# yangdongchao/Text-to-sound-Synthesis

Hardware: AMD Instinct MI355X
Metric: 10s clips/sec whole-node, 100-step Diffsound sample + VQ decode + vocoder (higher is better)
Workload: dtype f32 via 2-way fp16 split (3 MFMA passes, fp32 accumulate); 1 GPU; BASELINE configs[2]: full pipeline, batch 64 per GPU, 100 diffusion steps, codebook 256: CLIP text tower -> 19-layer denoiser -> SpecVQGAN decode -> MelGAN 22 kHz; global_batch=64, n_layer=19, parallelism=caption-sharded x1

## Files before the change

### include/diffsound_hip.h

```cpp
#ifndef DIFFSOUND_HIP_H
#define DIFFSOUND_HIP_H
#include <stdint.h>
#ifdef __cplusplus
extern "C" {
#endif

typedef void* ds_stream_t;

int ds_version(void);
const char* ds_last_error_string(void);

enum { DS_LOAD_DENSE = 0, DS_LOAD_CONV2D = 1, DS_LOAD_CONV1D = 2, DS_LOAD_CONVT1D = 3 };
enum { DS_PRO_NONE = 0, DS_PRO_AFFINE = 1, DS_PRO_AFFINE_SWISH = 2, DS_PRO_LRELU = 3 };
enum { DS_ACT_NONE = 0, DS_ACT_GELU2 = 1, DS_ACT_TANH = 2 };
enum { DS_STORE_ROW = 0, DS_STORE_BATCH_T = 1, DS_STORE_CONVT = 2, DS_STORE_ATTN = 3 };

typedef struct ds_gemm_desc {
    const float* A;
    const float* W;
    const float* bias;
    const float* R;
    float* C;
    int32_t M, N, K;
    int32_t lda, ldw, ldc, ldr;
// ... 15 lines not shown
    int64_t a_plane, c_plane;
    void* attn_kv;
    int32_t attn_heads, attn_nkey;
    int64_t attn_qplane;
} ds_gemm_desc;

int ds_gemm(const ds_gemm_desc* d, ds_stream_t stream);
void ds_gemm_force_tile(int cfg);
int ds_gemm_f16x2(const ds_gemm_desc* d, ds_stream_t stream);
int ds_gemm_f16x2_multi(const ds_gemm_desc* descs, int n, int cfg, ds_stream_t stream);
int ds_conv2d_f16x2(const ds_gemm_desc* d, ds_stream_t stream);
void ds_gemm_f16x2_force_tile(int cfg);
int ds_gemm_f16x2_auto_tile(int M, int N, int groups);
void ds_gemm_f16x2_set_balance_slots(int slots);
int ds_gemm_f16x2_plan(int cfg, int M, int N, int store, int* m_off, int* nbig, int* nsmall);

int ds_embed(const int64_t* tokens, const float* emb, const float* pos, float* out, int M, int L, int D,
             ds_stream_t stream);
int ds_adaln(const float* x, float* y, int M, int L, int D, const float* table, const int64_t* t,
             ds_stream_t stream);
int ds_layernorm(const float* x, float* y, int M, int D, const float* gamma, const float* beta,
                 ds_stream_t stream);
int ds_attention(const float* q, int ldq, const float* k, int ldk, const float* v, int ldv, float* o, int ldo,
                 int B, int heads, int Lq, int Lk, float scale, ds_stream_t stream);

int ds_attention_ex(const float* q, int ldq, const float* k, int ldk, const float* v, int ldv, float* o, int ldo,
                    int B, int heads, int Lq, int Lk, float scale, int causal, int f16_round, ds_stream_t stream);
int ds_attention_f16x2(const float* q, int ldq, const float* k, int ldk, const float* v, int ldv, float* o, int ldo,
                       int B, int heads, int Lq, int Lk, float scale, ds_stream_t stream);
int ds_adaln_split(const float* x, void* yh, int M, int L, int D, const float* table, const int64_t* t,
                   ds_stream_t stream);
int ds_layernorm_split(const float* x, void* yh, int M, int D, const float* gamma, const float* beta,
                       ds_stream_t stream);
int ds_attention_f16x2_split(const float* q, int ldq, const float* k, int ldk, const float* v, int ldv, void* oh,
                             int ldo, int B, int heads, int Lq, int Lk, float scale, ds_stream_t stream);
int ds_attn_nkey(int Lk);
int ds_attention_f16x2_ready(const void* qh, long long q_plane, const void* kv_img, void* oh, int ldo, int B, int heads,
                             int Lq, int Lk, float scale, ds_stream_t stream);
int ds_attn_pack_kv(const float* kv, int ld, int v_col, void* img, int B, int heads, int Lk, ds_stream_t stream);
int ds_embed_f16(const int64_t* tokens, const float* emb, const float* pos, float* out, int M, int L, int D,
                 ds_stream_t stream);
int ds_layernorm_f16(const float* x, float* y, int M, int D, const float* gamma, const float* beta,
                     ds_stream_t stream);
int ds_l2norm_rows_f16(const float* x, float* y, int M, int D, ds_stream_t stream);

int ds_sample_tail(const float* logits, const int64_t* xt, const int64_t* t, const float* u, const float* sched,
                   int64_t* out_tokens, float* dbg_log_pred, float* dbg_trunc, float* dbg_post, int B, int L,
                   int K, int T, int initial, float trunc_r, ds_stream_t stream);

int ds_sample_tail_ex(const float* logits, const int64_t* xt, const int64_t* t, const float* u, const float* sched,
                      int64_t* out_tokens, float* dbg_log_pred, float* dbg_trunc, float* dbg_post, int B, int L,
                      int K, int T, int initial, float trunc_r, int trunc_k, ds_stream_t stream);

int ds_q_sample(const int64_t* x0, const int64_t* t, const float* u, const float* sched, int64_t* out_tokens, int B,
                int L, int K, int T, ds_stream_t stream);

int ds_philox_uniforms(const int64_t* gids, unsigned long long seed, int call, int rng_stream, float* u, int B, int L,
                       int K, ds_stream_t stream);
int ds_sample_tail_rng(const float* logits, const int64_t* xt, const int64_t* t, const int64_t* gids,
                       unsigned long long seed, int call, const float* sched, int64_t* out_tokens, int B, int L, int K,
                       int T, int initial, float trunc_r, int trunc_k, ds_stream_t stream);
int ds_q_sample_rng(const int64_t* x0, const int64_t* t, const int64_t* gids, unsigned long long seed, int call,
                    const float* sched, int64_t* out_tokens, int B, int L, int K, int T, ds_stream_t stream);

int ds_sample_tail_hold(const float* logits, const int64_t* xt, const int64_t* t, const float* u, const float* sched,
                        int64_t* out_tokens, float* dbg_log_pred, float* dbg_trunc, float* dbg_post, int B, int L, int K,
// ... 283 lines not shown
```

### text-to-sound-synthesis_amd/_lib.py

```python
import ctypes as C
import os

import torch

_HERE = os.path.dirname(os.path.abspath(__file__))
LIB_PATH = os.environ.get("DIFFSOUND_LIB") or os.path.join(_HERE, "libdiffsound_hip.so")

LOAD_DENSE, LOAD_CONV2D, LOAD_CONV1D, LOAD_CONVT1D = 0, 1, 2, 3
PRO_NONE, PRO_AFFINE, PRO_AFFINE_SWISH, PRO_LRELU = 0, 1, 2, 3
ACT_NONE, ACT_GELU2, ACT_TANH = 0, 1, 2
LEVEL_MEASURE, LEVEL_PEAK, LEVEL_RMS, LEVEL_LOUDNESS = 0, 1, 2, 3
PASTE_EQUAL_POWER, PASTE_LINEAR = 0, 1
STORE_ROW, STORE_BATCH_T, STORE_CONVT, STORE_ATTN = 0, 1, 2, 3
(LP_ADALN1, LP_W_QKV, LP_B_QKV, LP_W_PROJ1, LP_B_PROJ1, LP_ADALN2, LP_W_Q2, LP_B_Q2, LP_W_KV2, LP_B_KV2,
 LP_W_PROJ2, LP_B_PROJ2, LP_LN2_G, LP_LN2_B, LP_W_FC1, LP_B_FC1, LP_W_FC2, LP_B_FC2, LP_COUNT) = range(19)

_vp, _i32, _i64, _f = C.c_void_p, C.c_int32, C.c_int64, C.c_float


class GemmDesc(C.Structure):
    _fields_ = [("A", _vp), ("W", _vp), ("bias", _vp), ("R", _vp), ("C", _vp),
                ("M", _i32), ("N", _i32), ("K", _i32),
                ("lda", _i32), ("ldw", _i32), ("ldc", _i32), ("ldr", _i32),
                ("groups", _i32),
# ... 9 lines not shown

class DenoiserDesc(C.Structure):
    _fields_ = [("n_layer", _i32), ("n_embd", _i32), ("n_head", _i32), ("seq_len", _i32),
                ("cond_len", _i32), ("cond_dim", _i32), ("n_codes", _i32), ("n_steps", _i32),
                ("mlp_mult", _i32),
                ("tok_emb", _vp), ("pos_emb", _vp), ("lnf_g", _vp), ("lnf_b", _vp),
                ("w_logits", _vp), ("b_logits", _vp), ("sched", _vp)]


_PROTOS = {
    "ds_version": (C.c_int, []),
    "ds_last_error_string": (C.c_char_p, []),
    "ds_gemm": (C.c_int, [C.POINTER(GemmDesc), _vp]),
    "ds_gemm_force_tile": (None, [C.c_int]),
    "ds_gemm_f16x2": (C.c_int, [C.POINTER(GemmDesc), _vp]),
    "ds_conv2d_f16x2": (C.c_int, [C.POINTER(GemmDesc), _vp]),
    "ds_gemm_f16x2_multi": (C.c_int, [C.POINTER(GemmDesc), C.c_int, C.c_int, _vp]),
    "ds_gemm_f16x2_auto_tile": (C.c_int, [C.c_int, C.c_int, C.c_int]),
    "ds_gemm_f16x2_force_tile": (None, [C.c_int]),
    "ds_gemm_f16x2_set_balance_slots": (None, [C.c_int]),
    "ds_gemm_f16x2_plan": (C.c_int, [C.c_int, C.c_int, C.c_int, C.c_int, C.POINTER(C.c_int), C.POINTER(C.c_int), C.POINTER(C.c_int)]),
    "ds_denoiser_set_split_weights": (C.c_int, [_vp, C.c_int, C.POINTER(_vp), C.POINTER(_f), _vp, _f]),
    "ds_embed": (C.c_int, [_vp, _vp, _vp, _vp, C.c_int, C.c_int, C.c_int, _vp]),
    "ds_adaln": (C.c_int, [_vp, _vp, C.c_int, C.c_int, C.c_int, _vp, _vp, _vp]),
    "ds_layernorm": (C.c_int, [_vp, _vp, C.c_int, C.c_int, _vp, _vp, _vp]),
    "ds_attention": (C.c_int, [_vp, C.c_int, _vp, C.c_int, _vp, C.c_int, _vp, C.c_int,
                               C.c_int, C.c_int, C.c_int, C.c_int, _f, _vp]),
    "ds_attention_ex": (C.c_int, [_vp, C.c_int, _vp, C.c_int, _vp, C.c_int, _vp, C.c_int,
                                  C.c_int, C.c_int, C.c_int, C.c_int, _f, C.c_int, C.c_int, _vp]),
    "ds_attention_f16x2": (C.c_int, [_vp, C.c_int, _vp, C.c_int, _vp, C.c_int, _vp, C.c_int,
                                     C.c_int, C.c_int, C.c_int, C.c_int, _f, _vp]),
    "ds_adaln_split": (C.c_int, [_vp, _vp, C.c_int, C.c_int, C.c_int, _vp, _vp, _vp]),
    "ds_layernorm_split": (C.c_int, [_vp, _vp, C.c_int, C.c_int, _vp, _vp, _vp]),
    "ds_attention_f16x2_split": (C.c_int, [_vp, C.c_int, _vp, C.c_int, _vp, C.c_int, _vp, C.c_int,
                                           C.c_int, C.c_int, C.c_int, C.c_int, _f, _vp]),
    "ds_attn_nkey": (C.c_int, [C.c_int]),
    "ds_attention_f16x2_ready": (C.c_int, [_vp, _i64, _vp, _vp, C.c_int, C.c_int, C.c_int, C.c_int, C.c_int, _f, _vp]),
    "ds_attn_pack_kv": (C.c_int, [_vp, C.c_int, C.c_int, _vp, C.c_int, C.c_int, C.c_int, _vp]),
    "ds_embed_f16": (C.c_int, [_vp, _vp, _vp, _vp, C.c_int, C.c_int, C.c_int, _vp]),
    "ds_layernorm_f16": (C.c_int, [_vp, _vp, C.c_int, C.c_int, _vp, _vp, _vp]),
    "ds_l2norm_rows_f16": (C.c_int, [_vp, _vp, C.c_int, C.c_int, _vp]),
    "ds_sample_tail": (C.c_int, [_vp, _vp, _vp, _vp, _vp, _vp, _vp, _vp, _vp,
                                 C.c_int, C.c_int, C.c_int, C.c_int, C.c_int, _f, _vp]),
    "ds_sample_tail_ex": (C.c_int, [_vp, _vp, _vp, _vp, _vp, _vp, _vp, _vp, _vp,
                                    C.c_int, C.c_int, C.c_int, C.c_int, C.c_int, _f, C.c_int, _vp]),
    "ds_q_sample": (C.c_int, [_vp, _vp, _vp, _vp, _vp, C.c_int, C.c_int, C.c_int, C.c_int, _vp]),
    "ds_philox_uniforms": (C.c_int, [_vp, C.c_uint64, C.c_int, C.c_int, _vp, C.c_int, C.c_int, C.c_int, _vp]),
    "ds_sample_tail_rng": (C.c_int, [_vp, _vp, _vp, _vp, C.c_uint64, C.c_int, _vp, _vp, C.c_int, C.c_int, C.c_int, C.c_int,
                                     C.c_int, _f, C.c_int, _vp]),
    "ds_q_sample_rng": (C.c_int, [_vp, _vp, _vp, C.c_uint64, C.c_int, _vp, _vp, C.c_int, C.c_int, C.c_int, C.c_int, _vp]),
    "ds_vq_argmin": (C.c_int, [_vp, _vp, _vp, _vp, _vp, C.c_int, C.c_int, C.c_int, _vp]),
    "ds_loss_tail": (C.c_int, [_vp, _vp, _vp, _vp, _vp, _vp, _vp, _vp, _vp, C.c_int, C.c_int, C.c_int, C.c_int, _vp]),
    "ds_loss_tail_bwd": (C.c_int, [_vp, _vp, _vp, _vp, _vp, _vp, _vp, C.c_int, C.c_int, C.c_int, C.c_int, _f, _f, _f,
                                   C.c_int, _vp]),
    "ds_layernorm_bwd": (C.c_int, [_vp, _vp, _vp, _vp, C.c_int, C.c_int, C.c_int, C.c_int, _vp, _vp, _vp, _vp]),
    "ds_layernorm_bwd_chunks": (C.c_int, [C.c_int, C.c_int, C.c_int]),
    "ds_layernorm_bwd_sums": (C.c_int, [_vp, _vp, _vp, _vp, C.c_int, C.c_int, C.c_int, C.c_int, _vp, _vp, _vp, C.c_int, _vp]),
    "ds_colsum": (C.c_int, [_vp, _vp, C.c_int, C.c_int, C.c_int, _i64, _i64, C.c_int, _vp]),
    "ds_colsum_ws": (C.c_int, [_vp, _vp, C.c_int, C.c_int, C.c_int, _i64, _i64, C.c_int, _vp, _i64, _vp]),
    "ds_gelu2": (C.c_int, [_vp, _vp, _vp, _i64, _vp]),
    "ds_softmax_bwd_rows": (C.c_int, [_vp, _vp, C.c_int, C.c_int, C.c_int, _f, _vp]),
    "ds_attention_bwd": (C.c_int, [_vp, C.c_int, _vp, C.c_int, _vp, C.c_int, _vp, C.c_int, _vp, C.c_int, _vp, C.c_int,
                                   _vp, C.c_int, _vp, C.c_int, _vp, C.c_int, C.c_int, C.c_int, C.c_int, _f, _vp]),
    "ds_attention_bwd_f16x2": (C.c_int, [_vp, C.c_int, _vp, C.c_int, _vp, C.c_int, _vp, C.c_int, _vp, C.c_int, _vp, C.c_int,
                                   _vp, C.c_int, _vp, C.c_int, _vp, C.c_int, C.c_int, C.c_int, C.c_int, _f, _vp]),
    "ds_attention_bwd_f16x2_mon": (C.c_int, [_vp, C.c_int, _vp, C.c_int, _vp, C.c_int, _vp, C.c_int, _vp, C.c_int, _vp, C.c_int,
# ... 275 lines not shown
```

### text-to-sound-synthesis_amd/csrc/api.hip

```cpp
#include <stdarg.h>
#include <stdio.h>
#include <string.h>

#include <vector>

#include "sampler.h"

static thread_local char g_err[512] = "";

void ds_set_error(const char* fmt, ...) {
    va_list ap;
    va_start(ap, fmt);
    vsnprintf(g_err, sizeof(g_err), fmt, ap);
    va_end(ap);
}

extern "C" int ds_version(void) { return 100; }
extern "C" const char* ds_last_error_string(void) { return g_err; }

static void fill(GemmParams& p, const ds_gemm_desc* d) {
    p.A = d->A; p.W = d->W; p.bias = d->bias; p.R = d->R; p.C = d->C;
    p.M = d->M; p.N = d->N; p.K = d->K;
    p.lda = d->lda; p.ldw = d->ldw > 0 ? d->ldw : d->K; p.ldc = d->ldc; p.ldr = d->ldr;
    p.groups = d->groups > 0 ? d->groups : 1;
// ... 93 lines not shown
    DS_CHECK_ARG(w_logits3, "missing split logits weight");
    h->lp3.assign(split3, split3 + (size_t)h->d.n_layer * DS_LP_COUNT);
    h->osc.assign(out_scales, out_scales + (size_t)h->d.n_layer * DS_LP_COUNT);
    h->w_logits3 = w_logits3;
    h->logits_osc = logits_scale;
    h->split_mode = mode;
    return 0;
}

extern "C" int ds_denoiser_create(const ds_denoiser_desc* desc, const void* const* layer_ptrs, ds_denoiser** out) {
    DS_CHECK_ARG(desc && layer_ptrs && out, "null pointer");
    DS_CHECK_ARG(desc->n_embd == 1024 && desc->n_embd == desc->n_head * 64, "built for n_embd 1024, head dim 64");
    DS_CHECK_ARG(desc->n_codes == 256 || desc->n_codes == 512, "codebook size must be 256 or 512");
    DS_CHECK_ARG(desc->cond_dim % 32 == 0 && desc->cond_len <= 96 && desc->seq_len <= 288, "unsupported lengths");
    DS_CHECK_ARG(desc->tok_emb && desc->pos_emb && desc->lnf_g && desc->lnf_b && desc->w_logits && desc->b_logits &&
                     desc->sched,
                 "null weight pointer");
    for (int i = 0; i < desc->n_layer * DS_LP_COUNT; ++i) DS_CHECK_ARG(layer_ptrs[i], "null layer pointer");
    ds_denoiser* h = new ds_denoiser;
    h->d = *desc;
    h->lp.resize((size_t)desc->n_layer * DS_LP_COUNT);
    for (size_t i = 0; i < h->lp.size(); ++i) h->lp[i] = (const float*)layer_ptrs[i];
    *out = h;
    return 0;
}

extern "C" void ds_denoiser_destroy(ds_denoiser* h) { delete h; }

struct Carve {
    float *x, *hn, *qkv, *att, *fc, *logits;
    float* kvimg;
};
static size_t attn_img_floats(int B, int heads, int Lk) { return (size_t)B * heads * 4 * ds_attn_nkey(Lk) * 64 / 2; }
static const int PS_ROWS = 272;
bool ds_gemm_f16x2_ps_taken(int B, int N);
static int rows_per_sample(const ds_denoiser* h, int B) {
    const int L = h->d.seq_len;
    if (!h->pad_rows || h->split_mode != DS_SPLIT_F16X2 || L > PS_ROWS || L <= PS_ROWS - 16) return L;
    return ds_gemm_f16x2_ps_taken(B, h->d.n_embd) ? PS_ROWS : L;
}
extern "C" int ds_denoiser_rows_per_sample(const ds_denoiser* h, int B) { return h && B > 0 ? rows_per_sample(h, B) : -1; }
extern "C" int ds_denoiser_set_row_padding(ds_denoiser* h, int on) {
    DS_CHECK_ARG(h, "null handle");
    h->pad_rows = on != 0;
    return 0;
}

int ds_amax_packed_hi(const void* plane, int M, int K, float* out, ds_stream_t stream);
extern "C" int ds_denoiser_set_range_monitor(ds_denoiser* h, float* peak) {
    DS_CHECK_ARG(h, "null handle");
    h->range_peak = peak;
    return 0;
}

static size_t carve(const ds_denoiser* h, int B, void* ws, Carve* c, int Lp = 0) {
    const size_t M = (size_t)B * (Lp > 0 ? Lp : PS_ROWS > h->d.seq_len ? PS_ROWS : h->d.seq_len), D = h->d.n_embd;
    const size_t M16 = (M + 15) & ~(size_t)15;
    size_t off = 0;
    auto take = [&](size_t n) {
        float* p = ws ? (float*)ws + off : nullptr;
        off += (n + 63) & ~(size_t)63;
        return p;
    };
    Carve t;
    t.x = take(M * D);
    t.hn = take(M16 * D);
// ... 91 lines not shown
        int rc_ = (x);    \
        if (rc_) return rc_; \
    } while (0)

extern "C" int ds_denoiser_cond_kv(const ds_denoiser* h, const float* cond, int B, float* kv, ds_stream_t stream) {
    DS_CHECK_ARG(h && cond && kv && B > 0, "bad arguments");
    const int D = h->d.n_embd, Mc = B * h->d.cond_len;
    if (h->split_mode == DS_SPLIT_F16X2) {
        const size_t per = kv_layer_img_floats(h, B);
        float* rows = kv + (size_t)h->d.n_layer * per;
        for (int l = 0; l < h->d.n_layer; ++l) {
            TRY(dense(cond, h->d.cond_dim, h->P(l, DS_LP_W_KV2), h->P(l, DS_LP_B_KV2), nullptr, rows, 2 * D, Mc, 2 * D,
                      h->d.cond_dim, DS_ACT_NONE, (hipStream_t)stream));
            TRY(ds_attn_pack_kv(rows, 2 * D, D, kv + (size_t)l * per, B, h->d.n_head, h->d.cond_len, stream));
        }
        return 0;
    }
    for (int l = 0; l < h->d.n_layer; ++l)
        TRY(dense(cond, h->d.cond_dim, h->P(l, DS_LP_W_KV2), h->P(l, DS_LP_B_KV2), nullptr,
                  kv + (size_t)l * Mc * 2 * D, 2 * D, Mc, 2 * D, h->d.cond_dim, DS_ACT_NONE, (hipStream_t)stream));
    return 0;
}

static int forward_impl(const ds_denoiser* h, const int64_t* tokens, const int64_t* t, const float* kv, int B,
                        const Carve& w, float* logits, int layout, hipStream_t s, int Lp, bool zero_kv_pad = true) {
    const ds_denoiser_desc& d = h->d;
    const int D = d.n_embd, Lv = d.seq_len, L = Lp, M = B * L, Mc = B * d.cond_len, F = D * d.mlp_mult;
    DS_CHECK_ARG(Lp == Lv || (layout == 0 && Lp > Lv), "padded rows need the row-major logits layout");
    g_prof_row_frac = (double)Lv / Lp;
    const float scale = 0.125f;
    const bool f16 = h->split_mode == DS_SPLIT_F16X2;
    const long long M16 = (M + 15) & ~15;
    const long long pD = f16 ? M16 * D : 0, pF = f16 ? M16 * F : 0;
    auto adaln = [&](int l, int slot) {
        return f16 ? ds_adaln_split(w.x, w.hn, M, L, D, h->P(l, slot), t, s)
                   : ds_adaln(w.x, w.hn, M, L, D, h->P(l, slot), t, s);
    };
    auto lnorm = [&](const float* g, const float* b_) {
        return f16 ? ds_layernorm_split(w.x, w.hn, M, D, g, b_, s) : ds_layernorm(w.x, w.hn, M, D, g, b_, s);
    };
    auto attn = [&](const float* q, int ldq, const float* k, const float* v, int ldkv, int Lk) {
        return ds_attention(q, ldq, k, ldkv, v, ldkv, w.att, D, B, d.n_head, L, Lk, scale, s);
    };
    const long long qpl = (long long)M * D;
    const int nkS = ds_attn_nkey(L);
    auto lin_attn = [&](int l, int slot, int bslot, int N, int n_weight, void* imgs) {
        return dense(w.hn, D, h->P(l, slot), h->P(l, bslot), nullptr, w.qkv, N, M, N, D, DS_ACT_NONE, s, DS_STORE_ATTN, L,
                     h->P3(l, slot), h->split_mode, h->S3(l, slot), pD, 0, imgs, d.n_head, nkS, qpl,
                     (long long)n_weight * D);
    };
    auto attn_ready = [&](const void* imgs, int Lk) {
        return ds_attention_f16x2_ready(w.qkv, qpl, imgs, w.att, D, B, d.n_head, L, Lk, scale, s);
    };
    if (f16 && zero_kv_pad) {
        hipError_t e = hipMemsetAsync(w.kvimg, 0, attn_img_floats(B, d.n_head, L) * sizeof(float), s);
        if (e != hipSuccess) {
            ds_set_error("forward: hipMemsetAsync: %s", hipGetErrorString(e));
            return -2;
        }
    }
    auto lin = [&](int l, int slot, int bslot, const float* A, int lda, long long ap, const float* R, float* C, int N,
                   int K, int act, long long cp) {
        return dense(A, lda, h->P(l, slot), h->P(l, bslot), R, C, N, M, N, K, act, s, DS_STORE_ROW, L, h->P3(l, slot),
                     h->split_mode, h->S3(l, slot), ap, cp);
    };
    TRY(ds_embed_rows(tokens, d.tok_emb, d.pos_emb, w.x, B, Lv, L, D, s));
    for (int l = 0; l < d.n_layer; ++l) {
        TRY(adaln(l, DS_LP_ADALN1));
        if (f16) {
            TRY(lin_attn(l, DS_LP_W_QKV, DS_LP_B_QKV, 3 * D, 3 * D, w.kvimg));
            TRY(attn_ready(w.kvimg, Lv));
        } else {
// ... 371 lines not shown
```

### text-to-sound-synthesis_amd/csrc/gemm_f16x2_ps.hip

```cpp
#include <stdlib.h>

#include "common.h"


typedef _Float16 h8 __attribute__((ext_vector_type(8)));
typedef unsigned u32x4 __attribute__((ext_vector_type(4)));
typedef unsigned u32x2 __attribute__((ext_vector_type(2)));
typedef __attribute__((address_space(1))) const void* ds_gptr;
typedef __attribute__((address_space(3))) void* ds_lptr;

#define PS_HLD 32
#define PS_BM 288
#define PS_BN 256
#define PS_LEAD 6
#define PS_GM 4
#define PS_STAGE_BYTES (2 * 2 * (PS_BM + PS_BN) * PS_HLD * 2)
#define PS_EPI_BYTES (2 * 64 * (PS_BN + 4) * 4)
#ifndef PS_DIRECT_SPLIT
#define PS_DIRECT_SPLIT 1
#endif
#ifndef PS_DIRECT_QK
#define PS_DIRECT_QK 0
#endif
#define PS_LDS_BYTES (PS_EPI_BYTES > PS_STAGE_BYTES ? PS_EPI_BYTES : PS_STAGE_BYTES)
#define PS_SIG(q_) ((0x78 >> (2 * (q_))) & 3)

enum { PS_EPI_ROW = 0, PS_EPI_SPLIT = 1, PS_EPI_ATTN = 2 };

template <int EPI, bool NB16>
__global__ __launch_bounds__(512, 1) void ds_gemm_f16x2_ps_kernel(const GemmParams p) {
    extern __shared__ __attribute__((aligned(16))) unsigned char smem_raw[];
    constexpr int BM = PS_BM, BN = PS_BN, HLD = PS_HLD, LEAD = PS_LEAD;
    constexpr int APL = BM * HLD, BPL = BN * HLD, STAGE = 2 * (APL + BPL);
    _Float16* smem = (_Float16*)smem_raw;
    const int tid = threadIdx.x, lane = tid & 63, wave = tid >> 6, l31 = lane & 31, hh = lane >> 5;
    const int wr = wave >> 2, wc = wave & 3;
    const int L = p.rows_per_sample;
    const int tiles_n = p.N / BN, nblk = gridDim.x;
    int bid = blockIdx.x;
    {
        const int xcd = bid & 7, idx = bid >> 3, q = nblk >> 3, r = nblk & 7;
        bid = (xcd < r ? xcd * (q + 1) : r * (q + 1) + (xcd - r) * q) + idx;
    }
    int tm_, tn_;
    {
        const int tiles_m = p.M / L;
        const int per = PS_GM * tiles_n, grp = bid / per, first = grp * PS_GM;
        const int gsz = tiles_m - first < PS_GM ? tiles_m - first : PS_GM;
        const int in = bid - grp * per;
        tm_ = first + in % gsz;
        tn_ = in / gsz;
    }
    const int row_lo = tm_ * L;
    const int m0 = (row_lo >> 4) << 4, n0 = tn_ * BN;
    const int nk = p.K / 32;
    const _Float16* Ap = (const _Float16*)p.A;
    const _Float16* Wp = (const _Float16*)p.W;
    unsigned long long src[4][2], src8;
    int ldsoff[4][2], ldsoff8;
    const unsigned lane16 = lane * 16;
    const int rgsA = (p.M + 15) >> 4, rgsB = (p.N + 15) >> 4;
#define PS_BASE(dst_, ptr_)                                                                          \
    do {                                                                                             \
        const unsigned long long a_ = (unsigned long long)(ptr_);                                    \
        dst_ = ((unsigned long long)(unsigned)__builtin_amdgcn_readfirstlane((unsigned)(a_ >> 32)) << 32) | \
               (unsigned long long)(unsigned)__builtin_amdgcn_readfirstlane((unsigned)a_);           \
    } while (0)
#pragma unroll
    for (int ty = 0; ty < 4; ++ty)
#pragma unroll
        for (int k = 0; k < 2; ++k) {
            const int idx = 2 * wave + k, plane = idx >> 3, r = idx & 7;
            const bool isA = (ty == 0 || ty == 3);
            const int s = isA ? (ty == 3) : (ty == 2);
            const int gip = isA ? (r >> 2) * 8 + s * 4 + (r & 3)
                                : (r >> 1) * 4 + s * 2 + (r & 1);
            int rg = ((isA ? m0 : n0) >> 4) + gip;
            const int rgs = isA ? rgsA : rgsB;
            if (rg >= rgs) rg = rgs - 1;
            PS_BASE(src[ty][k], (isA ? Ap + plane * p.a_plane : Wp + plane * p.w3_plane) + (size_t)rg * nk * 512);
            ldsoff[ty][k] = __builtin_amdgcn_readfirstlane((isA ? plane * 18 + gip : 36 + plane * 16 + gip) * 1024);
        }
    {
        const int e = wave & 3, plane = e >> 1, gip = 16 + (e & 1);
        int rg = (m0 >> 4) + gip;
        if (rg >= rgsA) rg = rgsA - 1;
        PS_BASE(src8, Ap + plane * p.a_plane + (size_t)rg * nk * 512);
        ldsoff8 = __builtin_amdgcn_readfirstlane((plane * 18 + gip) * 1024);
    }
#define PS_ISSUE(tile_, ty_, buf_)                                                                   \
    do {                                                                                             \
        _Pragma("unroll") for (int k = 0; k < 2; ++k)                                                \
            __builtin_amdgcn_global_load_lds((ds_gptr)((const unsigned char*)(src[ty_][k] + (unsigned long long)(tile_) * 1024) + lane16), \
                                             (ds_lptr)(smem_raw + (buf_) * (STAGE * 2) + ldsoff[ty_][k]), 16, 0, 0); \
        if ((ty_) == 3)                                                                              \
            __builtin_amdgcn_global_load_lds((ds_gptr)((const unsigned char*)(src8 + (unsigned long long)(tile_) * 1024) + lane16), \
                                             (ds_lptr)(smem_raw + (buf_) * (STAGE * 2) + ldsoff8), 16, 0, 0); \
    } while (0)
#define PS_DMA_ASM(base_, lds_, stage_)                                                              \
    do {                                                                                             \
        asm volatile("s_add_u32 m0, %2, %3\n\ts_nop 0\n\tglobal_load_lds_dwordx4 %0, %1"            \
                     :: "v"(lane16), "s"(base_), "s"(lds_), "n"(stage_) : "memory", "scc", "m0");    \
        base_ += 1024;                                                                               \
    } while (0)
#define PS_ISSUE_LOOP(tq_, ty_, buf_)                                                                \
    do {                                                                                             \
        PS_DMA_ASM(cur[ty_][0], ldsabs[ty_][0], (buf_) * (STAGE * 2));                               \
        PS_DMA_ASM(cur[ty_][1], ldsabs[ty_][1], (buf_) * (STAGE * 2));                               \
        if ((ty_) == 3) PS_DMA_ASM(cur8, ldsabs8, (buf_) * (STAGE * 2));                             \
    } while (0)
#define PS_FENCE()                                                                                   \
    do { asm volatile("" ::: "memory"); __builtin_amdgcn_sched_barrier(0); } while (0)
#define PS_BAR()                                                                                     \
    do { PS_FENCE(); __builtin_amdgcn_s_barrier(); PS_FENCE(); } while (0)
#define PS_LBAR() PS_BAR()
    const int swz[2] = {((0 + hh) ^ ((l31 >> 2) & 3)) * 8, ((2 + hh) ^ ((l31 >> 2) & 3)) * 8};
    f32x16 acc[4][2], acc8;
    f32x4 acc9[2];
#pragma unroll
    for (int r = 0; r < 16; ++r) acc8[r] = 0.f;
#pragma unroll
    for (int tt = 0; tt < 2; ++tt) acc9[tt] = f32x4{0.f, 0.f, 0.f, 0.f};
#pragma unroll
    for (int i = 0; i < 4; ++i)
#pragma unroll
        for (int j = 0; j < 2; ++j)
#pragma unroll
            for (int r = 0; r < 16; ++r) acc[i][j][r] = 0.f;
    h8 a0[2][2], a1[2][2];
    h8 b0[2][2], b1[2][2];
    h8 e0[2], e1[2];
    h8 ea0, ea1, eb0[2], eb1[2];
    const int l15 = PS_SIG((lane >> 2) & 3) * 4 + (lane & 3);
    const int swzq = ((lane >> 4) ^ ((l15 >> 2) & 3)) * 8;
#define PS_READ_A(buf_, s_)                                                                          \
    do {                                                                                             \
        const _Float16* Ac = smem + (buf_) * STAGE + (wr * 128 + (s_) * 64 + l31) * HLD;             \
        _Pragma("unroll") for (int ks = 0; ks < 2; ++ks)                                             \
            _Pragma("unroll") for (int ib = 0; ib < 2; ++ib) {                                       \
                a0[ks][ib] = *(const h8*)(Ac + ib * 32 * HLD + swz[ks]);                             \
                a1[ks][ib] = *(const h8*)(Ac + APL + ib * 32 * HLD + swz[ks]);                       \
            }                                                                                        \
// ... 404 lines not shown
```

### text-to-sound-synthesis_amd/csrc/norm.hip

```cpp
#include "common.h"

__device__ __forceinline__ float wave_sum(float v) {
#pragma unroll
    for (int o = 32; o > 0; o >>= 1) v += __shfl_xor(v, o);
    return v;
}
__device__ __forceinline__ double wave_sum_d(double v) {
#pragma unroll
    for (int o = 32; o > 0; o >>= 1) v += __shfl_xor(v, o);
    return v;
}

__global__ __launch_bounds__(256) void ds_embed_kernel(const int64_t* __restrict__ tok,
                                                       const float* __restrict__ emb,
                                                       const float* __restrict__ pos,
                                                       float* __restrict__ out, int M, int L, int D, int f16, int Lp) {
    const int row = blockIdx.x * 4 + (threadIdx.x >> 6);
    if (row >= M) return;
    const int lane = threadIdx.x & 63;
    const int b = row / Lp, ps = row - b * Lp;
    float* o = out + (size_t)row * D;
    if (ps >= L) {
        for (int c = lane * 4; c < D; c += 256) *(f32x4*)(o + c) = f32x4{0.f, 0.f, 0.f, 0.f};
        return;
    }
    long long t = tok[(size_t)b * L + ps];
    if (t < 0) t = 0;
    const float* e = emb + (size_t)t * D;
    const float* p = pos + (size_t)ps * D;
    for (int c = lane * 4; c < D; c += 256) {
        const f32x4 a = *(const f32x4*)(e + c), b = *(const f32x4*)(p + c);
        f32x4 r = a + b;
        if (f16) {
#pragma unroll
            for (int k = 0; k < 4; ++k) r[k] = ds_r16(ds_r16(a[k]) + ds_r16(b[k]));
        }
        *(f32x4*)(o + c) = r;
    }
}

template <int D>
__global__ __launch_bounds__(256) void ds_layernorm_kernel(const float* __restrict__ x, float* __restrict__ y,
                                                           int M, int L, int mode,
                                                           const float* __restrict__ tab,
                                                           const int64_t* __restrict__ t,
                                                           const float* __restrict__ gamma,
                                                           const float* __restrict__ beta, float eps, int f16) {
    const int row = blockIdx.x * 4 + (threadIdx.x >> 6);
    if (row >= M) return;
    const int lane = threadIdx.x & 63;
    constexpr int NV = D / 256;
    f32x4 v[NV];
    const float* xr = x + (size_t)row * D;
    float s = 0.f;
#pragma unroll
    for (int j = 0; j < NV; ++j) {
        v[j] = *(const f32x4*)(xr + (j * 64 + lane) * 4);
        s += (v[j][0] + v[j][1]) + (v[j][2] + v[j][3]);
    }
    const float mean = wave_sum(s) * (1.f / D);
    float q = 0.f;
#pragma unroll
    for (int j = 0; j < NV; ++j) {
#pragma unroll
        for (int k = 0; k < 4; ++k) {
            const float d = v[j][k] - mean;
            q += d * d;
        }
    }
    const float rstd = 1.f / sqrtf(wave_sum(q) * (1.f / D) + eps);
    const float *sc, *sh;
    if (mode == 0) {
        const long long tt = t[row / L];
        sc = tab + (size_t)tt * 2 * D;
        sh = sc + D;
    } else {
        sc = gamma;
        sh = beta;
    }
    float* yr = y + (size_t)row * D;
#pragma unroll
    for (int j = 0; j < NV; ++j) {
        const int c = (j * 64 + lane) * 4;
        const f32x4 a = *(const f32x4*)(sc + c), b = *(const f32x4*)(sh + c);
        f32x4 o;
#pragma unroll
        for (int k = 0; k < 4; ++k) {
            const float xn = (v[j][k] - mean) * rstd;
            o[k] = mode == 0 ? xn * (1.f + a[k]) + b[k] : xn * a[k] + b[k];
            if (f16 == 1) o[k] = ds_r16(o[k]);
        }
        if (f16 == 2) {
            typedef _Float16 h4 __attribute__((ext_vector_type(4)));
            h4 hi, lo;
#pragma unroll
            for (int k = 0; k < 4; ++k) {
                hi[k] = ds_split_hi(o[k]);
                lo[k] = ds_split_lo(o[k], hi[k]);
            }
            _Float16* yh = (_Float16*)y + ds_packed_off(row, c, D / 32);
            *(h4*)yh = hi;
            *(h4*)(yh + (size_t)((M + 15) & ~15) * D) = lo;
        } else {
            *(f32x4*)(yr + c) = o;
        }
    }
// ... 80 lines not shown
        const double ga = gamma[c], be = beta[c];
        scale[(size_t)b * C + c] = (float)(rstd * ga);
        shift[(size_t)b * C + c] = (float)(be - mean * rstd * ga);
    }
}

extern "C" int ds_embed(const int64_t* tokens, const float* emb, const float* pos, float* out, int M, int L,
                        int D, ds_stream_t stream_) {
    hipStream_t stream = (hipStream_t)stream_;
    DS_CHECK_ARG(tokens && emb && pos && out, "null pointer");
    DS_CHECK_ARG(M > 0 && L > 0 && D % 4 == 0, "bad shape");
    hipLaunchKernelGGL(ds_embed_kernel, dim3((M + 3) / 4), dim3(256), 0, stream, tokens, emb, pos, out, M, L, D, 0, L);
    DS_CHECK_LAUNCH();
    return 0;
}

int ds_embed_rows(const int64_t* tokens, const float* emb, const float* pos, float* out, int B, int L, int Lp,
                             int D, ds_stream_t stream_) {
    hipStream_t stream = (hipStream_t)stream_;
    DS_CHECK_ARG(tokens && emb && pos && out, "null pointer");
    DS_CHECK_ARG(B > 0 && L > 0 && Lp >= L && D % 4 == 0, "bad shape");
    const int M = B * Lp;
    hipLaunchKernelGGL(ds_embed_kernel, dim3((M + 3) / 4), dim3(256), 0, stream, tokens, emb, pos, out, M, L, D, 0, Lp);
    DS_CHECK_LAUNCH();
    return 0;
}

extern "C" int ds_adaln(const float* x, float* y, int M, int L, int D, const float* table, const int64_t* t,
                        ds_stream_t stream_) {
    hipStream_t stream = (hipStream_t)stream_;
    DS_CHECK_ARG(x && y && table && t, "null pointer");
    DS_CHECK_ARG(D == 1024, "only D = 1024 is built");
    hipLaunchKernelGGL((ds_layernorm_kernel<1024>), dim3((M + 3) / 4), dim3(256), 0, stream, x, y, M, L, 0, table,
                       t, (const float*)nullptr, (const float*)nullptr, 1e-5f, 0);
    DS_CHECK_LAUNCH();
    return 0;
}

extern "C" int ds_layernorm(const float* x, float* y, int M, int D, const float* gamma, const float* beta,
                            ds_stream_t stream_) {
    hipStream_t stream = (hipStream_t)stream_;
    DS_CHECK_ARG(x && y && gamma && beta, "null pointer");
    DS_CHECK_ARG(D == 1024, "only D = 1024 is built");
    hipLaunchKernelGGL((ds_layernorm_kernel<1024>), dim3((M + 3) / 4), dim3(256), 0, stream, x, y, M, 1, 1,
                       (const float*)nullptr, (const int64_t*)nullptr, gamma, beta, 1e-5f, 0);
    DS_CHECK_LAUNCH();
    return 0;
}

extern "C" int ds_groupnorm_stats(const float* x, int B, int P, int C, int groups, const float* gamma,
                                  const float* beta, float eps, double* work, float* scale, float* shift,
                                  ds_stream_t stream_) {
    hipStream_t stream = (hipStream_t)stream_;
    DS_CHECK_ARG(x && gamma && beta && work && scale && shift, "null pointer");
    DS_CHECK_ARG(B > 0 && P > 0 && C > 0, "sizes must be positive");
    DS_CHECK_ARG(groups > 0 && groups <= 64 && C % groups == 0, "bad group count");
    DS_CHECK_ARG(C % 4 == 0 && C <= 1024 && ((uintptr_t)x & 15) == 0, "C % 4 == 0, C <= 1024, 16-byte aligned x");
    const int nchunk = (P + GN_PCHUNK - 1) / GN_PCHUNK;
    hipLaunchKernelGGL(ds_gn_partial_kernel, dim3(nchunk, B), dim3(256), 0, stream, x, work, P, C, C / groups);
    DS_CHECK_LAUNCH();
    hipLaunchKernelGGL(ds_gn_finish_kernel, dim3(groups, B), dim3(256), 0, stream, work, nchunk, P, C, groups, gamma, beta,
                       eps, scale, shift, x);
    DS_CHECK_LAUNCH();
    return 0;
}

extern "C" int ds_groupnorm_finish(const double* part, int B, int nchunk, int P, int C, int groups, const float* gamma,
                                   const float* beta, float eps, float* scale, float* shift, ds_stream_t stream_) {
    hipStream_t stream = (hipStream_t)stream_;
    DS_CHECK_ARG(part && gamma && beta && scale && shift, "null pointer");
    DS_CHECK_ARG(B > 0 && nchunk > 0 && P > 0 && C > 0 && groups > 0 && groups <= 64 && C % groups == 0, "bad shape / group count");
    hipLaunchKernelGGL(ds_gn_finish_kernel, dim3(groups, B), dim3(256), 0, stream, part, nchunk, P, C, groups, gamma, beta, eps,
                       scale, shift, (const float*)nullptr);
    DS_CHECK_LAUNCH();
    return 0;
}

extern "C" int ds_embed_f16(const int64_t* tokens, const float* emb, const float* pos, float* out, int M, int L,
                            int D, ds_stream_t stream_) {
    hipStream_t stream = (hipStream_t)stream_;
    DS_CHECK_ARG(tokens && emb && pos && out, "null pointer");
    DS_CHECK_ARG(M > 0 && L > 0 && D % 4 == 0, "bad shape");
    hipLaunchKernelGGL(ds_embed_kernel, dim3((M + 3) / 4), dim3(256), 0, stream, tokens, emb, pos, out, M, L, D, 1, L);
    DS_CHECK_LAUNCH();
    return 0;
}

extern "C" int ds_layernorm_f16(const float* x, float* y, int M, int D, const float* gamma, const float* beta,
                                ds_stream_t stream_) {
    hipStream_t stream = (hipStream_t)stream_;
    DS_CHECK_ARG(x && y && gamma && beta, "null pointer");
    DS_CHECK_ARG(D == 512 || D == 1024, "D must be 512 or 1024");
    if (D == 512)
        hipLaunchKernelGGL((ds_layernorm_kernel<512>), dim3((M + 3) / 4), dim3(256), 0, stream, x, y, M, 1, 1,
                           (const float*)nullptr, (const int64_t*)nullptr, gamma, beta, 1e-5f, 1);
    else
        hipLaunchKernelGGL((ds_layernorm_kernel<1024>), dim3((M + 3) / 4), dim3(256), 0, stream, x, y, M, 1, 1,
                           (const float*)nullptr, (const int64_t*)nullptr, gamma, beta, 1e-5f, 1);
    DS_CHECK_LAUNCH();
    return 0;
}

__global__ __launch_bounds__(256) void ds_l2norm_rows_kernel(const float* __restrict__ x, float* __restrict__ y, int M,
                                                             int D) {
    const int row = blockIdx.x * 4 + (threadIdx.x >> 6);
    if (row >= M) return;
    const int lane = threadIdx.x & 63;
    const float* xr = x + (size_t)row * D;
    float s = 0.f;
    for (int c = lane; c < D; c += 64) s += xr[c] * xr[c];
    const float n = ds_r16(sqrtf(wave_sum(s)));
    float* yr = y + (size_t)row * D;
    for (int c = lane; c < D; c += 64) yr[c] = ds_r16(xr[c] / n);
}

extern "C" int ds_l2norm_rows_f16(const float* x, float* y, int M, int D, ds_stream_t stream_) {
    hipStream_t stream = (hipStream_t)stream_;
    DS_CHECK_ARG(x && y && M > 0 && D > 0, "bad arguments");
    hipLaunchKernelGGL(ds_l2norm_rows_kernel, dim3((M + 3) / 4), dim3(256), 0, stream, x, y, M, D);
    DS_CHECK_LAUNCH();
    return 0;
}

extern "C" int ds_adaln_split(const float* x, void* yh, int M, int L, int D, const float* table, const int64_t* t,
                              ds_stream_t stream_) {
    hipStream_t stream = (hipStream_t)stream_;
    DS_CHECK_ARG(x && yh && table && t, "null pointer");
    DS_CHECK_ARG(D == 1024, "only D = 1024 is built");
    hipLaunchKernelGGL((ds_layernorm_kernel<1024>), dim3((M + 3) / 4), dim3(256), 0, stream, x, (float*)yh, M, L, 0,
                       table, t, (const float*)nullptr, (const float*)nullptr, 1e-5f, 2);
    DS_CHECK_LAUNCH();
    return 0;
}

extern "C" int ds_layernorm_split(const float* x, void* yh, int M, int D, const float* gamma, const float* beta,
                                  ds_stream_t stream_) {
    hipStream_t stream = (hipStream_t)stream_;
    DS_CHECK_ARG(x && yh && gamma && beta, "null pointer");
    DS_CHECK_ARG(D == 1024, "only D = 1024 is built");
    hipLaunchKernelGGL((ds_layernorm_kernel<1024>), dim3((M + 3) / 4), dim3(256), 0, stream, x, (float*)yh, M, 1, 1,
                       (const float*)nullptr, (const int64_t*)nullptr, gamma, beta, 1e-5f, 2);
    DS_CHECK_LAUNCH();
    return 0;
}
```

Before: 22.95 clips/s.

## Zero padded rows in split layernorm and load GEMM A tail once

Measured after the change: 23.06 clips/s, median of 6. No clear change (+0.4%).

```diff
diff --git a/include/diffsound_hip.h b/include/diffsound_hip.h
--- a/include/diffsound_hip.h
+++ b/include/diffsound_hip.h
@@ -71,6 +71,10 @@
                    ds_stream_t stream);
 int ds_layernorm_split(const float* x, void* yh, int M, int D, const float* gamma, const float* beta,
                        ds_stream_t stream);
+int ds_adaln_split_rows(const float* x, void* yh, int M, int Lp, int Lv, int D, const float* table, const int64_t* t,
+                        ds_stream_t stream);
+int ds_layernorm_split_rows(const float* x, void* yh, int M, int Lp, int Lv, int D, const float* gamma, const float* beta,
+                            ds_stream_t stream);
 int ds_attention_f16x2_split(const float* q, int ldq, const float* k, int ldk, const float* v, int ldv, void* oh,
                              int ldo, int B, int heads, int Lq, int Lk, float scale, ds_stream_t stream);
 int ds_attn_nkey(int Lk);
diff --git a/text-to-sound-synthesis_amd/_lib.py b/text-to-sound-synthesis_amd/_lib.py
--- a/text-to-sound-synthesis_amd/_lib.py
+++ b/text-to-sound-synthesis_amd/_lib.py
@@ -65,6 +65,8 @@
                                      C.c_int, C.c_int, C.c_int, C.c_int, _f, _vp]),
     "ds_adaln_split": (C.c_int, [_vp, _vp, C.c_int, C.c_int, C.c_int, _vp, _vp, _vp]),
     "ds_layernorm_split": (C.c_int, [_vp, _vp, C.c_int, C.c_int, _vp, _vp, _vp]),
+    "ds_adaln_split_rows": (C.c_int, [_vp, _vp, C.c_int, C.c_int, C.c_int, C.c_int, _vp, _vp, _vp]),
+    "ds_layernorm_split_rows": (C.c_int, [_vp, _vp, C.c_int, C.c_int, C.c_int, C.c_int, _vp, _vp, _vp]),
     "ds_attention_f16x2_split": (C.c_int, [_vp, C.c_int, _vp, C.c_int, _vp, C.c_int, _vp, C.c_int,
                                            C.c_int, C.c_int, C.c_int, C.c_int, _f, _vp]),
     "ds_attn_nkey": (C.c_int, [C.c_int]),
diff --git a/text-to-sound-synthesis_amd/csrc/api.hip b/text-to-sound-synthesis_amd/csrc/api.hip
--- a/text-to-sound-synthesis_amd/csrc/api.hip
+++ b/text-to-sound-synthesis_amd/csrc/api.hip
@@ -149,6 +149,9 @@
     float* kvimg;
 };
 static size_t attn_img_floats(int B, int heads, int Lk) { return (size_t)B * heads * 4 * ds_attn_nkey(Lk) * 64 / 2; }
+#ifndef DS_PAD_ZERO_NORM
+#define DS_PAD_ZERO_NORM 1
+#endif
 static const int PS_ROWS = 272;
 bool ds_gemm_f16x2_ps_taken(int B, int N);
 static int rows_per_sample(const ds_denoiser* h, int B) {
@@ -306,12 +309,15 @@
     const bool f16 = h->split_mode == DS_SPLIT_F16X2;
     const long long M16 = (M + 15) & ~15;
     const long long pD = f16 ? M16 * D : 0, pF = f16 ? M16 * F : 0;
+    const bool pad0 = DS_PAD_ZERO_NORM && f16 && L > Lv;
     auto adaln = [&](int l, int slot) {
-        return f16 ? ds_adaln_split(w.x, w.hn, M, L, D, h->P(l, slot), t, s)
-                   : ds_adaln(w.x, w.hn, M, L, D, h->P(l, slot), t, s);
+        return pad0 ? ds_adaln_split_rows(w.x, w.hn, M, L, Lv, D, h->P(l, slot), t, s)
+               : f16 ? ds_adaln_split(w.x, w.hn, M, L, D, h->P(l, slot), t, s)
+                     : ds_adaln(w.x, w.hn, M, L, D, h->P(l, slot), t, s);
     };
     auto lnorm = [&](const float* g, const float* b_) {
-        return f16 ? ds_layernorm_split(w.x, w.hn, M, D, g, b_, s) : ds_layernorm(w.x, w.hn, M, D, g, b_, s);
+        return pad0 ? ds_layernorm_split_rows(w.x, w.hn, M, L, Lv, D, g, b_, s)
+               : f16 ? ds_layernorm_split(w.x, w.hn, M, D, g, b_, s) : ds_layernorm(w.x, w.hn, M, D, g, b_, s);
     };
     auto attn = [&](const float* q, int ldq, const float* k, const float* v, int ldkv, int Lk) {
         return ds_attention(q, ldq, k, ldkv, v, ldkv, w.att, D, B, d.n_head, L, Lk, scale, s);
diff --git a/text-to-sound-synthesis_amd/csrc/gemm_f16x2_ps.hip b/text-to-sound-synthesis_amd/csrc/gemm_f16x2_ps.hip
--- a/text-to-sound-synthesis_amd/csrc/gemm_f16x2_ps.hip
+++ b/text-to-sound-synthesis_amd/csrc/gemm_f16x2_ps.hip
@@ -21,6 +21,9 @@
 #endif
 #ifndef PS_DIRECT_QK
 #define PS_DIRECT_QK 0
+#endif
+#ifndef PS_TAIL_ONCE
+#define PS_TAIL_ONCE 1
 #endif
 #define PS_LDS_BYTES (PS_EPI_BYTES > PS_STAGE_BYTES ? PS_EPI_BYTES : PS_STAGE_BYTES)
 #define PS_SIG(q_) ((0x78 >> (2 * (q_))) & 3)
@@ -81,7 +84,14 @@
             PS_BASE(src[ty][k], (isA ? Ap + plane * p.a_plane : Wp + plane * p.w3_plane) + (size_t)rg * nk * 512);
             ldsoff[ty][k] = __builtin_amdgcn_readfirstlane((isA ? plane * 18 + gip : 36 + plane * 16 + gip) * 1024);
         }
-    {
+    constexpr bool TAIL16 = NB16 && PS_TAIL_ONCE;
+    if constexpr (TAIL16) {
+        const int plane = wave >> 2, piece = wave & 3;
+        int rg = (m0 >> 4) + 16;
+        if (rg >= rgsA) rg = rgsA - 1;
+        PS_BASE(src8, (const unsigned char*)(Ap + plane * p.a_plane + (size_t)rg * nk * 512) + piece * 256);
+        ldsoff8 = __builtin_amdgcn_readfirstlane((plane * 18 + 16) * 1024 + piece * 256);
+    } else {
         const int e = wave & 3, plane = e >> 1, gip = 16 + (e & 1);
         int rg = (m0 >> 4) + gip;
         if (rg >= rgsA) rg = rgsA - 1;
@@ -93,7 +103,7 @@
         _Pragma("unroll") for (int k = 0; k < 2; ++k)                                                \
             __builtin_amdgcn_global_load_lds((ds_gptr)((const unsigned char*)(src[ty_][k] + (unsigned long long)(tile_) * 1024) + lane16), \
                                              (ds_lptr)(smem_raw + (buf_) * (STAGE * 2) + ldsoff[ty_][k]), 16, 0, 0); \
-        if ((ty_) == 3)                                                                              \
+        if ((ty_) == 3 && (!TAIL16 || lane < 16))                                                    \
             __builtin_amdgcn_global_load_lds((ds_gptr)((const unsigned char*)(src8 + (unsigned long long)(tile_) * 1024) + lane16), \
                                              (ds_lptr)(smem_raw + (buf_) * (STAGE * 2) + ldsoff8), 16, 0, 0); \
     } while (0)
@@ -103,11 +113,22 @@
                      :: "v"(lane16), "s"(base_), "s"(lds_), "n"(stage_) : "memory", "scc", "m0");    \
         base_ += 1024;                                                                               \
     } while (0)
+#define PS_DMA16_ASM(base_, lds_, stage_)                                                            \
+    do {                                                                                             \
+        unsigned long long ex_;                                                                      \
+        asm volatile("s_add_u32 m0, %3, %4\n\ts_mov_b64 %0, exec\n\ts_mov_b64 exec, 0xffff\n\t"      \
+                     "global_load_lds_dwordx4 %1, %2\n\ts_mov_b64 exec, %0"                          \
+                     : "=&s"(ex_) : "v"(lane16), "s"(base_), "s"(lds_), "n"(stage_) : "memory", "scc", "m0"); \
+        base_ += 1024;                                                                               \
+    } while (0)
 #define PS_ISSUE_LOOP(tq_, ty_, buf_)                                                                \
     do {                                                                                             \
         PS_DMA_ASM(cur[ty_][0], ldsabs[ty_][0], (buf_) * (STAGE * 2));                               \
         PS_DMA_ASM(cur[ty_][1], ldsabs[ty_][1], (buf_) * (STAGE * 2));                               \
-        if ((ty_) == 3) PS_DMA_ASM(cur8, ldsabs8, (buf_) * (STAGE * 2));                             \
+        if ((ty_) == 3) {                                                                            \
+            if constexpr (TAIL16) PS_DMA16_ASM(cur8, ldsabs8, (buf_) * (STAGE * 2));                 \
+            else PS_DMA_ASM(cur8, ldsabs8, (buf_) * (STAGE * 2));                                    \
+        }                                                                                            \
     } while (0)
 #define PS_FENCE()                                                                                   \
     do { asm volatile("" ::: "memory"); __builtin_amdgcn_sched_barrier(0); } while (0)
diff --git a/text-to-sound-synthesis_amd/csrc/norm.hip b/text-to-sound-synthesis_amd/csrc/norm.hip
--- a/text-to-sound-synthesis_amd/csrc/norm.hip
+++ b/text-to-sound-synthesis_amd/csrc/norm.hip
@@ -39,17 +39,37 @@
     }
 }
 
-template <int D>
+template <int D, bool PADDED = false>
 __global__ __launch_bounds__(256) void ds_layernorm_kernel(const float* __restrict__ x, float* __restrict__ y,
                                                            int M, int L, int mode,
                                                            const float* __restrict__ tab,
                                                            const int64_t* __restrict__ t,
                                                            const float* __restrict__ gamma,
-                                                           const float* __restrict__ beta, float eps, int f16) {
-    const int row = blockIdx.x * 4 + (threadIdx.x >> 6);
-    if (row >= M) return;
+                                                           const float* __restrict__ beta, float eps, int f16,
+                                                           int Lv) {
     const int lane = threadIdx.x & 63;
     constexpr int NV = D / 256;
+    int row, smp = 0;
+    if constexpr (PADDED) {
+        const int ps = blockIdx.x * 4 + (threadIdx.x >> 6);
+        smp = blockIdx.y;
+        if (ps >= L) return;
+        row = smp * L + ps;
+        if (ps >= Lv) {
+            typedef _Float16 h4 __attribute__((ext_vector_type(4)));
+            const h4 z = {(_Float16)0.f, (_Float16)0.f, (_Float16)0.f, (_Float16)0.f};
+#pragma unroll
+            for (int j = 0; j < NV; ++j) {
+                _Float16* yh = (_Float16*)y + ds_packed_off(row, (j * 64 + lane) * 4, D / 32);
+                *(h4*)yh = z;
+                *(h4*)(yh + (size_t)((M + 15) & ~15) * D) = z;
+            }
+            return;
+        }
+    } else {
+        row = blockIdx.x * 4 + (threadIdx.x >> 6);
+        if (row >= M) return;
+    }
     f32x4 v[NV];
     const float* xr = x + (size_t)row * D;
     float s = 0.f;
@@ -71,7 +91,7 @@
     const float rstd = 1.f / sqrtf(wave_sum(q) * (1.f / D) + eps);
     const float *sc, *sh;
     if (mode == 0) {
-        const long long tt = t[row / L];
+        const long long tt = t[PADDED ? smp : row / L];
         sc = tab + (size_t)tt * 2 * D;
         sh = sc + D;
     } else {
@@ -218,7 +238,7 @@
     DS_CHECK_ARG(x && y && table && t, "null pointer");
     DS_CHECK_ARG(D == 1024, "only D = 1024 is built");
     hipLaunchKernelGGL((ds_layernorm_kernel<1024>), dim3((M + 3) / 4), dim3(256), 0, stream, x, y, M, L, 0, table,
-                       t, (const float*)nullptr, (const float*)nullptr, 1e-5f, 0);
+                       t, (const float*)nullptr, (const float*)nullptr, 1e-5f, 0, 0);
     DS_CHECK_LAUNCH();
     return 0;
 }
@@ -229,7 +249,7 @@
     DS_CHECK_ARG(x && y && gamma && beta, "null pointer");
     DS_CHECK_ARG(D == 1024, "only D = 1024 is built");
     hipLaunchKernelGGL((ds_layernorm_kernel<1024>), dim3((M + 3) / 4), dim3(256), 0, stream, x, y, M, 1, 1,
-                       (const float*)nullptr, (const int64_t*)nullptr, gamma, beta, 1e-5f, 0);
+                       (const float*)nullptr, (const int64_t*)nullptr, gamma, beta, 1e-5f, 0, 0);
     DS_CHECK_LAUNCH();
     return 0;
 }
@@ -279,10 +299,10 @@
     DS_CHECK_ARG(D == 512 || D == 1024, "D must be 512 or 1024");
     if (D == 512)
         hipLaunchKernelGGL((ds_layernorm_kernel<512>), dim3((M + 3) / 4), dim3(256), 0, stream, x, y, M, 1, 1,
-                           (const float*)nullptr, (const int64_t*)nullptr, gamma, beta, 1e-5f, 1);
+                           (const float*)nullptr, (const int64_t*)nullptr, gamma, beta, 1e-5f, 1, 0);
     else
         hipLaunchKernelGGL((ds_layernorm_kernel<1024>), dim3((M + 3) / 4), dim3(256), 0, stream, x, y, M, 1, 1,
-                           (const float*)nullptr, (const int64_t*)nullptr, gamma, beta, 1e-5f, 1);
+                           (const float*)nullptr, (const int64_t*)nullptr, gamma, beta, 1e-5f, 1, 0);
     DS_CHECK_LAUNCH();
     return 0;
 }
@@ -314,7 +334,7 @@
     DS_CHECK_ARG(x && yh && table && t, "null pointer");
     DS_CHECK_ARG(D == 1024, "only D = 1024 is built");
     hipLaunchKernelGGL((ds_layernorm_kernel<1024>), dim3((M + 3) / 4), dim3(256), 0, stream, x, (float*)yh, M, L, 0,
-                       table, t, (const float*)nullptr, (const float*)nullptr, 1e-5f, 2);
+                       table, t, (const float*)nullptr, (const float*)nullptr, 1e-5f, 2, 0);
     DS_CHECK_LAUNCH();
     return 0;
 }
@@ -325,7 +345,33 @@
     DS_CHECK_ARG(x && yh && gamma && beta, "null pointer");
     DS_CHECK_ARG(D == 1024, "only D = 1024 is built");
     hipLaunchKernelGGL((ds_layernorm_kernel<1024>), dim3((M + 3) / 4), dim3(256), 0, stream, x, (float*)yh, M, 1, 1,
-                       (const float*)nullptr, (const int64_t*)nullptr, gamma, beta, 1e-5f, 2);
-    DS_CHECK_LAUNCH();
-    return 0;
-}
+                       (const float*)nullptr, (const int64_t*)nullptr, gamma, beta, 1e-5f, 2, 0);
+    DS_CHECK_LAUNCH();
+    return 0;
+}
+
+extern "C" int ds_adaln_split_rows(const float* x, void* yh, int M, int Lp, int Lv, int D, const float* table,
+                                   const int64_t* t, ds_stream_t stream_) {
+    hipStream_t stream = (hipStream_t)stream_;
+    DS_CHECK_ARG(x && yh && table && t, "null pointer");
+    DS_CHECK_ARG(D == 1024, "only D = 1024 is built");
+    DS_CHECK_ARG(M > 0 && Lp > 0 && Lv > 0 && Lv <= Lp, "0 < valid rows <= rows per sample");
+    DS_CHECK_ARG(M % Lp == 0 && M / Lp <= 65535, "rows = samples x rows per sample, at most 65535 samples");
+    hipLaunchKernelGGL((ds_layernorm_kernel<1024, true>), dim3((Lp + 3) / 4, M / Lp), dim3(256), 0, stream, x, (float*)yh, M,
+                       Lp, 0, table, t, (const float*)nullptr, (const float*)nullptr, 1e-5f, 2, Lv);
+    DS_CHECK_LAUNCH();
+    return 0;
+}
+
+extern "C" int ds_layernorm_split_rows(const float* x, void* yh, int M, int Lp, int Lv, int D, const float* gamma,
+                                       const float* beta, ds_stream_t stream_) {
+    hipStream_t stream = (hipStream_t)stream_;
+    DS_CHECK_ARG(x && yh && gamma && beta, "null pointer");
+    DS_CHECK_ARG(D == 1024, "only D = 1024 is built");
+    DS_CHECK_ARG(M > 0 && Lp > 0 && Lv > 0 && Lv <= Lp, "0 < valid rows <= rows per sample");
+    DS_CHECK_ARG(M % Lp == 0 && M / Lp <= 65535, "rows = samples x rows per sample, at most 65535 samples");
+    hipLaunchKernelGGL((ds_layernorm_kernel<1024, true>), dim3((Lp + 3) / 4, M / Lp), dim3(256), 0, stream, x, (float*)yh, M,
+                       Lp, 1, (const float*)nullptr, (const int64_t*)nullptr, gamma, beta, 1e-5f, 2, Lv);
+    DS_CHECK_LAUNCH();
+    return 0;
+}
```
